# jirsat/wavenets

Measured on NVIDIA B200. Metric: audio samples/sec fwd+bwd WaveNet stack, higher is better.
Workload: dtype bf16

## Files before the change

### include/wavenet_b200.h

```cpp
#ifndef WAVENET_B200_H_
#define WAVENET_B200_H_

#include <stddef.h>
#include <stdint.h>

#ifdef __cplusplus
extern "C" {
#endif

typedef struct wn_handle wn_handle;

enum wn_status {
  WN_OK = 0,
  WN_ERR_VALUE = -1,
  WN_ERR_UNSUPPORTED = -2,
  WN_ERR_CUDA = -3,
  WN_ERR_STATE = -4
};

enum wn_activation { WN_ACT_LINEAR = 0, WN_ACT_RELU = 1, WN_ACT_LEAKY_RELU = 2, WN_ACT_TANH = 3, WN_ACT_SIGMOID = 4 };
enum wn_sampling { WN_CATEGORICAL = 0, WN_LOGISTIC = 1, WN_GAUSSIAN = 2 };
enum wn_precision {
  WN_FP32 = 0,
  WN_BF16 = 1
// ... 80 lines not shown
int wn_forward_ex(wn_handle* h, const float* x_dev, const float* cond_dev, int B, int T, int training, float* out_dev, void* stream);

int wn_loss_fn(wn_handle* h, const void* target_dev, int target_is_int64, const float* pred_dev, int B, int T, float* out_dev, void* stream);

int wn_train_step(wn_handle* h, const float* frames_dev, const float* cond_dev, int B, int T,
                  int n_replicas, float* loss_dev, void* stream);
int wn_test_step(wn_handle* h, const float* frames_dev, const float* cond_dev, int B, int T,
                 int n_replicas, float* loss_dev, void* stream);
int wn_train_step_host(wn_handle* h, const float* frames_host, const float* cond_host, int B, int T,
                       int n_replicas, float* loss_host);

int wn_nccl_unique_id(uint8_t* id128);
int wn_comm_init(wn_handle* h, const uint8_t* id128, int nranks, int rank);
int wn_comm_attach(wn_handle* h, void* nccl_comm , int nranks, int rank);
int wn_comm_fuse_allreduce(wn_handle* h, int on);
int wn_allreduce_grads(wn_handle* h, void* stream);
const char* wn_nccl_info(void);

int wn_layer_forward(wn_handle* h, int block, const float* x_dev, const float* cond_dev, int B, int T,
                     float* x_out_dev, float* skip_dev, void* stream);
int wn_layer_forward_ex(wn_handle* h, int block, const float* x_dev, const float* cond_dev, int B, int T, int training,
                        float* x_out_dev, float* skip_dev, void* stream);
int wn_layer_backward(wn_handle* h, int block, const float* dx_out_dev, const float* dskip_dev,
                      float* dx_dev, float* dcond_dev, void* stream);

int wn_debug_tensor(wn_handle* h, const char* name, int index, float* out_host, int64_t capacity);
int wn_debug_conv_gemm(const void* a_bf16_dev, int lda, int B, int T, int nseg, const int* shifts, int K,
                       const void* w_bf16_dev, int N, int N16, int tile, float* out_dev, void* stream);
int wn_debug_wgrad(const void* a_bf16_dev, int lda, const void* g_bf16_dev, int ldg, int B, int T, int nseg,
                   const int* shifts, int K, int N, float* out_dev, void* stream);
// ... 21 lines not shown
```

### wavenets_b200/_lib.py

```python
from __future__ import annotations

import ctypes as C
import os

WN_MAX_LIST = 8
WN_MAX_DILATIONS = 512

WN_OK, WN_ERR_VALUE, WN_ERR_UNSUPPORTED, WN_ERR_CUDA, WN_ERR_STATE = 0, -1, -2, -3, -4
ACTIVATIONS = {None: 0, 'linear': 0, 'relu': 1, 'leaky_relu': 2, 'tanh': 3, 'sigmoid': 4}
SAMPLING = {'categorical': 0, 'logistic': 1, 'gaussian': 2}
PRECISION = {'fp32': 0, 'float32': 0, 'bf16': 1, 'bfloat16': 1}

EXPORTS = [
  'wn_create', 'wn_destroy', 'wn_last_error', 'wn_receptive_field', 'wn_dilation', 'wn_num_params',
  'wn_param_count', 'wn_param_info', 'wn_params_dev', 'wn_grads_dev', 'wn_set_param', 'wn_get_param',
  'wn_get_grad', 'wn_params_changed', 'wn_quantize', 'wn_forward', 'wn_train_step', 'wn_test_step',
  'wn_train_step_host', 'wn_layer_forward', 'wn_layer_backward', 'wn_last_launch_count',
  'wn_fused_forward_blocks', 'wn_grouped_wgrad_tiles', 'wn_stack_forward_layers', 'wn_profile_begin', 'wn_profile_end', 'wn_profile_get', 'wn_build_info', 'wn_set_dropout_masks', 'wn_set_dropout_seed', 'wn_layer_forward_ex', 'wn_num_frames', 'wn_preprocess_frames', 'wn_inverse_mu_law', 'wn_one_hot', 'wn_sample_waveform', 'wn_sample_last_step', 'wn_generate', 'wn_adam_init', 'wn_clip_grads', 'wn_adam_step', 'wn_adam_state', 'wn_debug_conv_gemm', 'wn_debug_wgrad', 'wn_debug_bench',
  'wn_forward_ex', 'wn_loss_fn', 'wn_adam_restore', 'wn_nccl_unique_id', 'wn_comm_init', 'wn_comm_attach', 'wn_comm_fuse_allreduce',
  'wn_allreduce_grads', 'wn_nccl_info', 'wn_grouped_wgrad_info', 'wn_debug_tensor', 'wn_stack_backward_layers',
  'wn_allreduce_buckets',
]


class WnConfig(C.Structure):
  _fields_ = [
    ('kernel_size', C.c_int32), ('channels', C.c_int32), ('blocks', C.c_int32), ('layers_per_block', C.c_int32),
    ('activation', C.c_int32), ('conditioning', C.c_int32), ('n_mapping', C.c_int32),
    ('mapping_layers', C.c_int32 * WN_MAX_LIST), ('mapping_activation', C.c_int32), ('cond_in', C.c_int32),
    ('dilation_bound', C.c_int32), ('num_mixtures', C.c_int32), ('sampling_function', C.c_int32), ('bits', C.c_int32),
    ('skip_channels', C.c_int32), ('dilation_channels', C.c_int32), ('use_residual', C.c_int32), ('use_skip', C.c_int32),
    ('n_final', C.c_int32), ('final_layers_channels', C.c_int32 * WN_MAX_LIST),
    ('l2_reg_factor', C.c_float), ('dropout', C.c_float),
    ('n_dilations', C.c_int32), ('dilations', C.c_int32 * WN_MAX_DILATIONS),
# ... 36 lines not shown
  lib.wn_grads_dev.argtypes = [vp]
  lib.wn_grads_dev.restype = vp
  lib.wn_set_param.argtypes = [vp, i32, vp]
  lib.wn_get_param.argtypes = [vp, i32, vp]
  lib.wn_get_grad.argtypes = [vp, i32, vp]
  lib.wn_params_changed.argtypes = [vp, vp]
  lib.wn_quantize.argtypes = [vp, vp, i64, i32, vp]
  lib.wn_forward.argtypes = [vp, vp, vp, i32, i32, vp, vp]
  lib.wn_forward_ex.argtypes = [vp, vp, vp, i32, i32, i32, vp, vp]
  lib.wn_loss_fn.argtypes = [vp, vp, i32, vp, i32, i32, vp, vp]
  lib.wn_adam_restore.argtypes = [vp, vp, vp, i64]
  lib.wn_nccl_unique_id.argtypes = [vp]
  lib.wn_comm_init.argtypes = [vp, vp, i32, i32]
  lib.wn_comm_attach.argtypes = [vp, vp, i32, i32]
  lib.wn_comm_fuse_allreduce.argtypes = [vp, i32]
  lib.wn_allreduce_grads.argtypes = [vp, vp]
  lib.wn_nccl_info.restype = C.c_char_p
  lib.wn_train_step.argtypes = [vp, vp, vp, i32, i32, i32, vp, vp]
  lib.wn_test_step.argtypes = [vp, vp, vp, i32, i32, i32, vp, vp]
  lib.wn_train_step_host.argtypes = [vp, vp, vp, i32, i32, i32, vp]
  lib.wn_layer_forward.argtypes = [vp, i32, vp, vp, i32, i32, vp, vp, vp]
  lib.wn_layer_forward_ex.argtypes = [vp, i32, vp, vp, i32, i32, i32, vp, vp, vp]
  lib.wn_layer_backward.argtypes = [vp, i32, vp, vp, vp, vp, vp]
  lib.wn_last_launch_count.argtypes = [vp]
  lib.wn_last_launch_count.restype = i64
  lib.wn_fused_forward_blocks.argtypes = [vp]
  lib.wn_grouped_wgrad_tiles.argtypes = [vp, C.POINTER(C.c_int)]
  lib.wn_stack_forward_layers.argtypes = [vp]
  lib.wn_stack_backward_layers.argtypes = [vp]
  lib.wn_allreduce_buckets.argtypes = [vp]
# ... 46 lines not shown
```

### wavenets_b200/build.py

```python
from __future__ import annotations

import hashlib
import os
import subprocess
import sys

HERE = os.path.dirname(os.path.abspath(__file__))
CSRC = os.path.join(HERE, 'csrc')
LIB = os.path.join(HERE, 'libwavenet_b200.so')
STAMP = os.path.join(HERE, '.libwavenet_b200.stamp')
FLAVOURS = {'': [], 'precise': ['-DWN_PRECISE_MATH'], 'tl': ['-DTC_TIMELINE']}

SOURCES = ['wn_api.cu']
HEADERS = ['common.cuh', 'generate.cuh', 'epilogues.cuh', 'gemm_simt.cuh', 'gemm_tc.cuh', 'gemm_tc_block.cuh', 'gemm_tc_wgroup.cuh', 'gemm_tc_stack.cuh', 'gemm_tc_stack_bwd.cuh', 'tc_common.cuh', 'tc_epilogues.cuh', 'kernels_misc.cuh', 'nccl_dl.cuh',
           os.path.join('..', '..', 'include', 'wavenet_b200.h')]

NVCC_FLAGS = [
  '-gencode', 'arch=compute_100a,code=sm_100a', '-lineinfo', '-O3', '-std=c++17',
  '-Xcompiler', '-fPIC', '-shared', '--expt-relaxed-constexpr',
  '-Xptxas', '-v', '-ldl',
]


def _flags(flavour: str = ''):
  return NVCC_FLAGS + FLAVOURS[flavour] + os.environ.get('WN_NVCC_EXTRA', '').split()


def lib_path(flavour: str = '') -> str:
  return LIB if not flavour else os.path.join(HERE, f'libwavenet_b200_{flavour}.so')
# ... 39 lines not shown
```

### wavenets_b200/csrc/wn_api.cu

```cuda
#include <cuda_runtime.h>
#include <math.h>
#include <stdarg.h>
#include <stdio.h>
#include <stdlib.h>
#include <string.h>

#include <algorithm>
#include <string>
#include <vector>

#include "../../include/wavenet_b200.h"
#include "common.cuh"
#include "epilogues.cuh"
#include "gemm_simt.cuh"
#include "gemm_tc.cuh"
#include "gemm_tc_block.cuh"
#include "gemm_tc_wgroup.cuh"
#include "gemm_tc_stack.cuh"
#include "gemm_tc_stack_bwd.cuh"
#include "kernels_misc.cuh"
#include "generate.cuh"
#include "nccl_dl.cuh"

static thread_local char g_err[512] = "";
static void set_err(const char* fmt, ...) {
  va_list ap;
  va_start(ap, fmt);
  vsnprintf(g_err, sizeof(g_err), fmt, ap);
  va_end(ap);
}
extern "C" const char* wn_last_error(void) { return g_err; }
extern "C" const char* wn_build_info(void) {
  return "libwavenet_b200 sm_100a; fp32 FFMA tier + bf16 tcgen05/TMEM/TMA tier; built " __DATE__ " " __TIME__;
}
// ... 140 lines not shown
  size_t prof_used = 0;
  long long prof_launches = 0;
  TmapCache tmaps;
  struct StepGraph { const float* frames; const float* cond; int B, T, nrep; float* loss; bool train; int seen; long long launches; cudaGraphExec_t exec; };
  std::vector<StepGraph> graphs;
  int use_graphs = 1;
  cudaEvent_t ev_in = nullptr, ev_out = nullptr;
  cudaStream_t side_stream = nullptr;
  std::vector<cudaEvent_t> ev_blk_in, ev_blk_dz, ev_blk_done;
  int use_side = 1;
  int use_res_gemm = 1;
  int use_fused_fwd = 1;
  int stack_fwd_layers = 0;
  int use_stack_fwd = 1;
  std::vector<TcStackPlan> stack_plans;
  int use_stack_bwd = 2, stack_bwd_layers = 0;
  std::vector<TcStackBwdPlan> stack_bwd_plans;
  int tile_gate_bwd = 0, tile_dgrad = 0;
  int fused_fwd_launches = 0;
  int use_group_wgrad = 0;
  void* dz_all = nullptr;
  void* dx_all = nullptr;
  void* do_all = nullptr;
  std::vector<std::vector<void*>> dp_keep;
  struct WgPlan { int B, T; bool drop; bool sb; int nb; TcWgGroupPlan plan; };
  std::vector<WgPlan> wg_plans;
  std::vector<TcWgJobDesc> wg_jobs;
  int dskip_l2_last = 0;
  int wg_last_tiles = 0, wg_last_side = 0;
  int wg_last_partials = 0;
// ... 408 lines not shown
  cudaMemset(h->d_grads, 0, (size_t)h->n_scalars * 4);
  cudaMemset(h->pack.base, 0, pack_bytes);
  cudaMemset(h->ws.base, 0, ws_bytes);
  cudaMallocHost(&h->pin_frames, (size_t)h->maxB * (h->maxT + 1) * 4);
  cudaMallocHost(&h->pin_cond, (size_t)h->maxB * (c.cond_in > 0 ? c.cond_in : 1) * 4);
  cudaMallocHost(&h->pin_loss, 16);
  cudaStreamCreateWithFlags(&h->own_stream, cudaStreamNonBlocking);
  cudaEventCreateWithFlags(&h->ev_in, cudaEventDisableTiming);
  cudaEventCreateWithFlags(&h->ev_out, cudaEventDisableTiming);
  { const char* e = getenv("WN_CUDA_GRAPH"); if (e && e[0] == '0') h->use_graphs = 0; }
  { const char* e = getenv("WN_SIDE_STREAM"); if (e && e[0] == '0') h->use_side = 0; }
  if (env_res && env_res[0] == '0') h->use_res_gemm = 0;
  { const char* e = getenv("WN_TC_FUSED_FWD"); if (e && e[0] == '0') h->use_fused_fwd = 0; }
  { const char* e = getenv("WN_TC_STACK_FWD"); if (e && e[0] == '0') h->use_stack_fwd = 0; }
  { const char* e = getenv("WN_TC_STACK_BWD"); if (e) h->use_stack_bwd = atoi(e); }
  { const char* e = getenv("WN_TC_TILE_GATE_BWD"); if (e) h->tile_gate_bwd = atoi(e); }
  { const char* e = getenv("WN_TC_TILE_DGRAD"); if (e) h->tile_dgrad = atoi(e); }
  { const char* e = getenv("WN_TC_MERGED_FINISH"); if (e && e[0] == '1') h->use_merged_finish = 1; }
  { const char* e = getenv("WN_TC_BALANCE_GRID"); if (e) g_tc_balance_env = atoi(e); }
  { const char* e = getenv("WN_TC_DSKIP_LAST"); if (e) h->dskip_l2_last = atoi(e); }
  cudaStreamCreateWithFlags(&h->side_stream, cudaStreamNonBlocking);
  cudaEventCreateWithFlags(&h->ev_wg_side, cudaEventDisableTiming);
  {
    int lo = 0, hi = 0;
    cudaDeviceGetStreamPriorityRange(&lo, &hi);
    if (cudaStreamCreateWithPriority(&h->comm_stream, cudaStreamNonBlocking, hi) != cudaSuccess) {
      cudaGetLastError();
      cudaStreamCreateWithFlags(&h->comm_stream, cudaStreamNonBlocking);
    }
  }
// ... 640 lines not shown
    }
  }
  if (!stacked)
  for (int l = 0; l < h->L; ++l) {
    RET(block_forward<T>(h, st, l, cur, c.conditioning != 0, B, Tn));
    cur = h->xout[l];
  }
  const void* head_in = cur;
  int head_w = h->R;
  if (c.use_skip) {
    OuterLabel ol(h, "skip_sum");
    RET((skip_gemm<T, T>(h, st, 0, h->L, (T*)h->skipsum, h->Sp, h->bskip_sum, B, Tn)));
    head_in = h->skipsum;
    head_w = h->Sp;
  }
  OuterLabel ol_head(h, "head_fwd");
  for (size_t i = 0; i < h->head.size(); ++i) {
    const ConvP& hc = h->head[i];
    const bool last = i + 1 == h->head.size();
    GemmH g;
    g.B = B; g.T = Tn; g.N = hc.cout; g.nseg = 1;
    g.seg[0] = SegH{head_in, head_w, 0, hc.cin};
    fill_w(g, hc, false);
    if (!last) {
      typename EpiBiasActRes<T, T, sizeof(T) == 2>::Params ep{};
      ep.out = (T*)h->hact[i]; ep.ldo = hc.cout; ep.bias = P_(h, hc.b_idx); ep.act = c.activation; ep.N = hc.cout; ep.vec = vec_ok<T>(hc.cout);
      RET((run_conv_gemm<T, EpiBiasActRes<T, T, sizeof(T) == 2>>(h, st, CLS_GEMM, g, ep)));
      head_in = h->hact[i];
      head_w = hc.cout;
    } else {
      typename EpiBiasActRes<T, float, sizeof(T) == 2>::Params ep{};
      ep.out = h->logits; ep.ldo = h->ldl; ep.bias = P_(h, hc.b_idx); ep.act = ACT_LINEAR; ep.N = hc.cout; ep.vec = vec_ok<float>(h->ldl);
      RET((run_conv_gemm<T, EpiBiasActRes<T, float, sizeof(T) == 2>>(h, st, CLS_GEMM, g, ep)));
    }
  }
  return WN_OK;
}

template <class T>
static int loss_forward(wn_handle* h, cudaStream_t st, const float* frames, int B, int Tn, float scale, bool want_grad, float* probs, float* loss_out) {
  const wn_config& c = h->cfg;
  const long long rows = (long long)B * Tn;
  int nparts;
  {
    OuterLabel ol(h, "loss");
    LaunchScope ls(h, st, CLS_LOSS);
    if (c.sampling_function == WN_CATEGORICAL) {
      nparts = cdiv(rows, 8);
      if (h->Cout == 256 && h->ldl == 256 && h->ldd % 4 == 0)
        softmax_ce_reg_kernel<T, 2><<<nparts, 256, 0, st>>>(h->logits, frames, Tn, rows, c.bits, scale, want_grad ? (T*)h->dlogits : nullptr, h->ldd, probs,
                                                           loss_out ? h->loss_partial : nullptr);
      else
        softmax_ce_kernel<T><<<nparts, 256, 0, st>>>(h->logits, h->Cout, frames, Tn, rows, c.bits, scale, want_grad ? (T*)h->dlogits : nullptr, h->ldd,
                                                    probs, loss_out ? h->loss_partial : nullptr);
    } else {
      mixture_loss_launch<T>(st, &nparts, h->logits, h->ldl, c.num_mixtures, frames, Tn, rows, c.bits, c.sampling_function == WN_GAUSSIAN ? 2 : 1, scale,
                             want_grad ? (T*)h->dlogits : nullptr, h->ldd, loss_out ? h->loss_partial : nullptr, Tn + 1, 1, nullptr);
    }
  }
// ... 396 lines not shown
    g.seg[0] = SegH{dcur, dw, 0, (sizeof(T) == 2 && i + 1 == (int)h->head.size()) ? h->ldd : hc.cout};
    fill_w(g, hc, true);
    typename EpiActBwd<T, T>::Params ep{};
    ep.N = hc.cin; ep.add = nullptr;
    void* dst;
    if (i > 0) {
      dst = (dcur == h->dhA) ? h->dhB : h->dhA;
      ep.out = (T*)dst; ep.ldo = hc.cin; ep.y = (const T*)h->hact[i - 1]; ep.ldy = hc.cin; ep.act = c.activation; ep.vec = vec_ok<T>(hc.cin);
    } else if (cat) {
      dst = (T*)h->dcatA + h->R;
      ep.out = (T*)dst; ep.ldo = ldc; ep.y = nullptr; ep.act = ACT_LINEAR; ep.vec = vec_ok<T>(ldc);
    } else {
      dst = c.use_skip ? h->dskip : (group ? dx_of(h->L - 1) : h->dxA);
      ep.out = (T*)dst; ep.ldo = hc.cin; ep.y = nullptr; ep.act = ACT_LINEAR; ep.vec = vec_ok<T>(hc.cin);
    }
    RET((run_conv_gemm<T, EpiActBwd<T, T>>(h, st, CLS_GEMM, g, ep)));
    dcur = dst;
    dw = hc.cin;
  }
  const void* dxout;
  int ld_dx;
  if (cat) {
    CK(cudaMemcpy2DAsync((T*)h->dcatB + h->R, (size_t)ldc * sizeof(T), (const T*)h->dcatA + h->R, (size_t)ldc * sizeof(T), (size_t)h->S * sizeof(T),
                         (size_t)B * Tn, cudaMemcpyDeviceToDevice, st));
    const void* cur = nullptr;
    void* nxt = h->dcatB;
    for (int l = h->L - 1; l >= 0; --l) {
      const void* x_in = l > 0 ? h->xout[l - 1] : h->h0;
      const void* dsk = cur ? (const void*)((const T*)cur + h->R) : (const void*)((const T*)h->dcatA + h->R);
      BwdSide sd; const BwdSide* sdp = side_setup(h, st, l, use_side, &sd);
      RET(block_backward<T>(h, st, l, x_in, cur, ldc, dsk, ldc, nxt, ldc, B, Tn, l2coef, (l & 1) ? h->dz2 : h->dz, sdp));
// ... 464 lines not shown
                                       mse_dev ? h->loss_partial : nullptr);
  if (mse_dev) loss_finalize<<<1, 1024, 0, st>>>(h->loss_partial, nparts, 1.0f / (float)rows, nullptr, 0.f, mse_dev);
  CK(cudaGetLastError());
  return WN_OK;
}
extern "C" int wn_sample_waveform(wn_handle* h, const float* pred_dev, int B, int T, int deterministic, uint64_t seed, float* out_dev, void* stream) {
  RET(check_bt(h, B, T));
  if (!pred_dev || !out_dev || !h->cfg.has_head) { set_err("bad sample arguments"); return WN_ERR_VALUE; }
  CK(cudaSetDevice(h->cfg.device));
  return sample_common(h, pred_dev, h->Cout, 0, nullptr, B, T, deterministic, seed, out_dev, nullptr, (cudaStream_t)stream);
}
extern "C" int wn_sample_last_step(wn_handle* h, const float* frames_dev, int deterministic, uint64_t seed, float* out_dev, float* mse_dev, void* stream) {
  if (!h || !h->cfg.has_head || h->lastB < 1) { set_err("no train/test step to sample from"); return WN_ERR_STATE; }
  if (!out_dev) { set_err("bad sample arguments"); return WN_ERR_VALUE; }
  CK(cudaSetDevice(h->cfg.device));
  return sample_common(h, h->logits, h->ldl, 1, mse_dev ? frames_dev : nullptr, h->lastB, h->lastT, deterministic, seed, out_dev, mse_dev, (cudaStream_t)stream);
}

extern "C" int wn_adam_init(wn_handle* h, float lr, float beta1, float beta2, float eps, float clipnorm) {
  if (!h) { set_err("null handle"); return WN_ERR_VALUE; }
  if (lr < 0.f || beta1 < 0.f || beta1 >= 1.f || beta2 < 0.f || beta2 >= 1.f || eps <= 0.f || clipnorm < 0.f) { set_err("bad Adam hyper-parameters"); return WN_ERR_VALUE; }
  CK(cudaSetDevice(h->cfg.device));
  h->opt_lr = lr; h->opt_b1 = beta1; h->opt_b2 = beta2; h->opt_eps = eps; h->opt_clipnorm = clipnorm; h->opt_t = 0;
  const size_t bytes = (size_t)h->n_scalars * 4;
  if (!h->opt_m) {
    CK(cudaMalloc(&h->opt_m, bytes)); CK(cudaMalloc(&h->opt_v, bytes));
    std::vector<OptChunk> ch; std::vector<int> first;
    for (size_t v = 0; v < h->params.size(); ++v) {
      first.push_back((int)ch.size());
      for (long long o = 0; o < h->params[v].count; o += OPT_CHUNK)
// ... 208 lines not shown
}
extern "C" int wn_comm_attach(wn_handle* h, void* nccl_comm, int nranks, int rank) {
  if (!h || nranks < 1) { set_err("bad communicator arguments"); return WN_ERR_VALUE; }
  char err[256];
  if (nccl_comm && nccl_load(err, sizeof(err)) != 0) { set_err("%s", err); return WN_ERR_CUDA; }
  if (h->comm && h->comm_owned) g_nccl.CommDestroy(h->comm);
  h->comm = (wn_ncclComm_t)nccl_comm; h->comm_owned = false; h->comm_nranks = nccl_comm ? nranks : 1; h->comm_rank = rank;
  drop_graphs_fwd(h);
  return WN_OK;
}
extern "C" int wn_comm_fuse_allreduce(wn_handle* h, int on) {
  if (!h) { set_err("null handle"); return WN_ERR_VALUE; }
  if ((on != 0) != (h->ar_in_step != 0)) { h->ar_in_step = on ? 1 : 0; drop_graphs_fwd(h); }
  return WN_OK;
}
extern "C" int wn_allreduce_grads(wn_handle* h, void* stream) {
  if (!h) { set_err("null handle"); return WN_ERR_VALUE; }
  if (h->comm_nranks <= 1) return WN_OK;
  CK(cudaSetDevice(h->cfg.device));
  return allreduce_grads(h, (cudaStream_t)stream);
}
extern "C" const char* wn_nccl_info(void) {
  static char buf[400];
  char err[256];
  if (nccl_load(err, sizeof(err)) != 0) { snprintf(buf, sizeof(buf), "unavailable: %s", err); return buf; }
  int v = 0;
  if (g_nccl.GetVersion) g_nccl.GetVersion(&v);
  snprintf(buf, sizeof(buf), "NCCL %d from %s", v, g_nccl.where);
  return buf;
}

template <class T>
static int step_entry(wn_handle* h, const float* frames, const float* cond, int B, int Tn, int nrep, float* loss, cudaStream_t st, bool train) {
  const float scale = 1.0f / ((float)B * (float)nrep);
  h->drop_active = train && h->cfg.dropout > 0.f;
  draw_dropout_masks(h, st, B, Tn);
  RET(model_forward<T>(h, st, frames, Tn + 1, cond, B, Tn));
  RET(loss_forward<T>(h, st, frames, B, Tn, scale, train, nullptr, loss));
  if (train) {
    const float l2coef = h->cfg.l2_reg_factor > 0.f ? 2.0f * h->cfg.l2_reg_factor / (float)nrep : 0.f;
    h->ar_now = h->ar_in_step && h->comm && h->comm_nranks > 1 && nrep > 1;
    RET(model_backward<T>(h, st, frames, Tn + 1, cond, B, Tn, l2coef));
    if (h->ar_now) RET(allreduce_grads(h, st));
    h->ar_now = false;
  }
  return WN_OK;
}

static int step_common(wn_handle* h, const float* frames_dev, const float* cond_dev, int B, int T, int n_replicas, float* loss_dev, void* stream, bool train) {
  RET(check_bt(h, B, T));
  if (!h->cfg.has_head || !h->cfg.has_input_conv) { set_err("train/test step needs a full model handle"); return WN_ERR_STATE; }
  if (h->cfg.conditioning && !cond_dev) { set_err("Conditioning must be provided."); return WN_ERR_VALUE; }
  if (n_replicas < 1 || !frames_dev || !loss_dev) { set_err("bad step arguments"); return WN_ERR_VALUE; }
  if (train && h->cfg.dropout >= 1.f) { set_err("dropout must be < 1 for training"); return WN_ERR_VALUE; }
  CK(cudaSetDevice(h->cfg.device));
  cudaStream_t st = (cudaStream_t)stream;
  auto run = [&](cudaStream_t s) -> int {
    h->launches = 0;
    return h->cfg.precision == WN_BF16 ? step_entry<bf16>(h, frames_dev, cond_dev, B, T, n_replicas, loss_dev, s, train)
                                       : step_entry<float>(h, frames_dev, cond_dev, B, T, n_replicas, loss_dev, s, train);
  };
  if (h->use_graphs && h->prof_tag == 0) {
    wn_handle::StepGraph* sg = nullptr;
    for (auto& g : h->graphs)
      if (g.frames == frames_dev && g.cond == cond_dev && g.B == B && g.T == T && g.nrep == n_replicas && g.loss == loss_dev && g.train == train) { sg = &g; break; }
    if (!sg) {
      if (h->graphs.size() >= 8) { for (auto& g : h->graphs) if (g.exec) cudaGraphExecDestroy(g.exec); h->graphs.clear(); }
      h->graphs.push_back({frames_dev, cond_dev, B, T, n_replicas, loss_dev, train, 0, 0, nullptr});
      sg = &h->graphs.back();
    }
    const bool legacy = st == nullptr || st == cudaStreamLegacy;
    cudaStream_t gs = legacy ? h->own_stream : st;
    if (sg->seen >= 1 && !sg->exec) {
      cudaGraph_t graph = nullptr;
      if (cudaStreamBeginCapture(gs, cudaStreamCaptureModeThreadLocal) == cudaSuccess) {
        int r = run(gs);
// ... 5 lines not shown
          h->use_graphs = 0;
          cudaGetLastError();
        }
        if (graph) cudaGraphDestroy(graph);
      } else {
        h->use_graphs = 0;
        cudaGetLastError();
      }
    }
    if (sg->exec) {
      if (legacy) { CK(cudaEventRecord(h->ev_in, st)); CK(cudaStreamWaitEvent(gs, h->ev_in, 0)); }
      CK(cudaGraphLaunch(sg->exec, gs));
      if (legacy) { CK(cudaEventRecord(h->ev_out, gs)); CK(cudaStreamWaitEvent(st, h->ev_out, 0)); }
      h->launches = sg->launches;
      h->lastB = B; h->lastT = T;
      return WN_OK;
    }
    sg->seen++;
  }
  RET(run(st));
  CK(cudaGetLastError());
  h->lastB = B; h->lastT = T;
  return WN_OK;
}

extern "C" int wn_train_step(wn_handle* h, const float* frames_dev, const float* cond_dev, int B, int T, int n_replicas, float* loss_dev, void* stream) {
  return step_common(h, frames_dev, cond_dev, B, T, n_replicas, loss_dev, stream, true);
}
extern "C" int wn_test_step(wn_handle* h, const float* frames_dev, const float* cond_dev, int B, int T, int n_replicas, float* loss_dev, void* stream) {
  return step_common(h, frames_dev, cond_dev, B, T, n_replicas, loss_dev, stream, false);
}

extern "C" int wn_train_step_host(wn_handle* h, const float* frames_host, const float* cond_host, int B, int T, int n_replicas, float* loss_host) {
  RET(check_bt(h, B, T));
  if (!frames_host || !loss_host) { set_err("bad step arguments"); return WN_ERR_VALUE; }
  CK(cudaSetDevice(h->cfg.device));
  cudaStream_t st = h->own_stream;
// ... 126 lines not shown
  const size_t rows_cap = (size_t)h->maxB * h->maxT;
  const bool bf = h->cfg.precision == WN_BF16;
  const size_t es = bf ? 2 : 4;
  const std::string n(name);
  const void* src = nullptr; int width = 0, ld = 0; bool f32 = false;
  const bool lok = index >= 0 && index < h->L;
  if (n == "h0") { src = h->h0; width = ld = h->R; }
  else if (n == "z" && lok) { src = h->zbuf[index]; width = ld = 2 * h->D; }
  else if (n == "g" && lok) { src = (const char*)h->G_all + (size_t)index * rows_cap * h->D * es; width = ld = h->D; }
  else if (n == "xout" && lok) { src = h->xout[index]; width = ld = h->R; }
  else if (n == "skipsum") { src = h->skipsum; width = ld = h->Sp; }
  else if (n == "hact" && index >= 0 && index < (int)h->hact.size()) { src = h->hact[index]; width = ld = h->head[index].cout; }
  else if (n == "act" && index >= 0 && index / 16 < h->L && index % 16 < (int)h->acts[index / 16].size()) {
    src = h->acts[index / 16][index % 16]; width = ld = h->D;
  }
  else if (n == "logits") { src = h->logits; width = h->Cout; ld = h->ldl; f32 = true; }
  else if (n == "dlogits") { src = h->dlogits; width = h->Cout; ld = h->ldd; }
  else if (n == "dskip") { src = h->dskip; width = ld = h->Sp; }
  else if (n == "dz" && lok && h->dz_all) { src = (const char*)h->dz_all + (size_t)index * rows_cap * 2 * h->D * es; width = ld = 2 * h->D; }
  else if (n == "dx" && lok && h->dx_all) { src = (const char*)h->dx_all + (size_t)index * rows_cap * h->R * es; width = ld = h->R; }
  if (!src || rows < 1) { set_err("debug_tensor: no tensor '%s'[%d] in this handle / step", name, index); return WN_ERR_STATE; }
  if ((long long)capacity < rows * width) { set_err("debug_tensor: capacity %lld < %lld", (long long)capacity, rows * width); return WN_ERR_VALUE; }
  const size_t e2 = f32 ? 4 : es;
  std::vector<char> tmp((size_t)rows * ld * e2);
  CK(cudaMemcpy(tmp.data(), src, tmp.size(), cudaMemcpyDeviceToHost));
  for (long long r = 0; r < rows; ++r)
    for (int c = 0; c < width; ++c) {
      const char* p = tmp.data() + ((size_t)r * ld + c) * e2;
      float v;
      if (e2 == 4) memcpy(&v, p, 4);
      else { uint16_t u; memcpy(&u, p, 2); uint32_t w = (uint32_t)u << 16; memcpy(&v, &w, 4); }
// ... 139 lines not shown
```

### wavenets_b200/model.py

```python
from __future__ import annotations

import ctypes as C
import math
import warnings
from typing import Optional

import numpy as np
import torch

from . import _lib
from ._engine import Handle, as_dev
from .layers import WaveNetLayer
from .metrics import Mean


class _PendingLogs:

  def __init__(self, model, slot, event):
    self._model, self._slot, self._event, self._out = model, slot, event, None

  def result(self):
    if self._out is None:
      self._event.synchronize()
      m = self._model
# ... 75 lines not shown
    self.dilations = [kernel_size ** (i % max_power) for i in range(layers_per_block * blocks)]
    self.receptive_field = 1 + sum(self.dilations) * (kernel_size - 1) + 1

    self._act = _lib.activation_code(activation)
    self._map_act = _lib.activation_code(mapping_activation)
    self.optimizer = None
    self.built = False
    self._handle: Optional[Handle] = None
    self._pending_weights = None
    self._staging = {}
    self._metrics_from_compilation = []
    self.loss_tracker = None
    self.reg_loss = None
    self.last_step_logs = {}
    self._sample_seed, self._sample_calls = 0x42, 0
    self._pin_logs, self._pin_events, self._pending_slot = None, None, 0
    self._last_frames, self._last_rows = None, 0
    self.n_replicas = 1
    self.replica_rank = 0
    self._process_group = None
    self._comm = None
    self._dropout_seed = 0x243F6A8885A308D3
    self._ar_fused = False

  def compile(self, **kwargs):
    if 'loss' in kwargs:
      raise ValueError('Loss must be set in the model init function.')
    self.optimizer = kwargs.get('optimizer', None)
    self._metrics_from_compilation = list(kwargs.get('metrics') or [])
    self.loss_tracker = Mean(name='loss')
# ... 199 lines not shown
    dev = torch.device('cuda', self.device_index)
    if len(x.shape) == 3 and x.shape[2] != 1:
      raise ValueError('input must be (batch, samples, 1)')
    B, T = int(x.shape[0]), int(x.shape[1]) - 1
    frames = self._stage('frames', x, (B, T + 1), dev)
    cond = self._stage('cond', cond, (B, int(cond.shape[-1])), dev) if cond is not None else None
    self._ensure_built(frames[:, :-1], cond)
    h = self.handle
    self._last_frames, self._last_rows = frames, B * T
    fn = h.lib.wn_train_step if train else h.lib.wn_test_step
    if train and self._comm is not None:
      fuse = not (self.optimizer is not None and getattr(self.optimizer, 'clipnorm', None))
      if fuse != self._ar_fused:
        _lib.check(h.lib.wn_comm_fuse_allreduce(h.h, 1 if fuse else 0))
        self._ar_fused = fuse
    _lib.check(fn(h.h, h.ptr(frames), h.ptr(cond), B, T, self.n_replicas, h.ptr(h._loss), h.stream_ptr()))
    clip = train and self.optimizer is not None and getattr(self.optimizer, 'clipnorm', None)
    if clip:
      self.optimizer.clip(self)
    if train and self.n_replicas > 1:
      if self._comm is not None:
        if not self._ar_fused:
          _lib.check(h.lib.wn_allreduce_grads(h.h, h.stream_ptr()))
      elif self._process_group is not None:
        torch.distributed.all_reduce(h.flat_grads, op=torch.distributed.ReduceOp.SUM, group=self._process_group)
    return h._loss[:2]

  def train_step(self, data):
    loss = self._step(data, True)
    if self.optimizer is not None:
# ... 163 lines not shown
```

Before: 11.03 million.

## Fuse head forward, categorical loss and head backward into one tcgen05 kernel

Adds a persistent 2-CTA cluster kernel that runs the three 1x1 head convolutions, the softmax cross-entropy loss with its gradient, and the backward head GEMMs in one launch. Intermediates stay in TMEM and shared memory, and only bf16 outputs are stored through TMA. This removes separate GEMM and loss launches and the fp32 logits round trip. Logits are no longer written by default; they are recomputed lazily when sampling, debugging or metrics need them, which adds state-tracking complexity.

```diff
diff --git a/include/wavenet_b200.h b/include/wavenet_b200.h
--- a/include/wavenet_b200.h
+++ b/include/wavenet_b200.h
@@ -118,6 +118,7 @@
 int wn_comm_init(wn_handle* h, const uint8_t* id128, int nranks, int rank);
 int wn_comm_attach(wn_handle* h, void* nccl_comm , int nranks, int rank);
 int wn_comm_fuse_allreduce(wn_handle* h, int on);
+int wn_keep_logits(wn_handle* h, int on);
 int wn_allreduce_grads(wn_handle* h, void* stream);
 const char* wn_nccl_info(void);
 
diff --git a/wavenets_b200/_lib.py b/wavenets_b200/_lib.py
--- a/wavenets_b200/_lib.py
+++ b/wavenets_b200/_lib.py
@@ -17,7 +17,7 @@
   'wn_get_grad', 'wn_params_changed', 'wn_quantize', 'wn_forward', 'wn_train_step', 'wn_test_step',
   'wn_train_step_host', 'wn_layer_forward', 'wn_layer_backward', 'wn_last_launch_count',
   'wn_fused_forward_blocks', 'wn_grouped_wgrad_tiles', 'wn_stack_forward_layers', 'wn_profile_begin', 'wn_profile_end', 'wn_profile_get', 'wn_build_info', 'wn_set_dropout_masks', 'wn_set_dropout_seed', 'wn_layer_forward_ex', 'wn_num_frames', 'wn_preprocess_frames', 'wn_inverse_mu_law', 'wn_one_hot', 'wn_sample_waveform', 'wn_sample_last_step', 'wn_generate', 'wn_adam_init', 'wn_clip_grads', 'wn_adam_step', 'wn_adam_state', 'wn_debug_conv_gemm', 'wn_debug_wgrad', 'wn_debug_bench',
-  'wn_forward_ex', 'wn_loss_fn', 'wn_adam_restore', 'wn_nccl_unique_id', 'wn_comm_init', 'wn_comm_attach', 'wn_comm_fuse_allreduce',
+  'wn_forward_ex', 'wn_loss_fn', 'wn_adam_restore', 'wn_nccl_unique_id', 'wn_comm_init', 'wn_comm_attach', 'wn_comm_fuse_allreduce', 'wn_keep_logits',
   'wn_allreduce_grads', 'wn_nccl_info', 'wn_grouped_wgrad_info', 'wn_debug_tensor', 'wn_stack_backward_layers',
   'wn_allreduce_buckets',
 ]
@@ -84,6 +84,7 @@
   lib.wn_comm_init.argtypes = [vp, vp, i32, i32]
   lib.wn_comm_attach.argtypes = [vp, vp, i32, i32]
   lib.wn_comm_fuse_allreduce.argtypes = [vp, i32]
+  lib.wn_keep_logits.argtypes = [vp, i32]
   lib.wn_allreduce_grads.argtypes = [vp, vp]
   lib.wn_nccl_info.restype = C.c_char_p
   lib.wn_train_step.argtypes = [vp, vp, vp, i32, i32, i32, vp, vp]
diff --git a/wavenets_b200/build.py b/wavenets_b200/build.py
--- a/wavenets_b200/build.py
+++ b/wavenets_b200/build.py
@@ -12,7 +12,7 @@
 FLAVOURS = {'': [], 'precise': ['-DWN_PRECISE_MATH'], 'tl': ['-DTC_TIMELINE']}
 
 SOURCES = ['wn_api.cu']
-HEADERS = ['common.cuh', 'generate.cuh', 'epilogues.cuh', 'gemm_simt.cuh', 'gemm_tc.cuh', 'gemm_tc_block.cuh', 'gemm_tc_wgroup.cuh', 'gemm_tc_stack.cuh', 'gemm_tc_stack_bwd.cuh', 'tc_common.cuh', 'tc_epilogues.cuh', 'kernels_misc.cuh', 'nccl_dl.cuh',
+HEADERS = ['common.cuh', 'generate.cuh', 'epilogues.cuh', 'gemm_simt.cuh', 'gemm_tc.cuh', 'gemm_tc_block.cuh', 'gemm_tc_wgroup.cuh', 'gemm_tc_stack.cuh', 'gemm_tc_stack_bwd.cuh', 'gemm_tc_head.cuh', 'tc_common.cuh', 'tc_epilogues.cuh', 'kernels_misc.cuh', 'nccl_dl.cuh',
            os.path.join('..', '..', 'include', 'wavenet_b200.h')]
 
 NVCC_FLAGS = [
diff --git a/wavenets_b200/csrc/gemm_tc_head.cuh b/wavenets_b200/csrc/gemm_tc_head.cuh
--- /dev/null
+++ b/wavenets_b200/csrc/gemm_tc_head.cuh
@@ -0,0 +1,365 @@
+#pragma once
+#include "gemm_tc_block.cuh"
+#include "kernels_misc.cuh"
+
+struct TcHeadMaps {
+  CUtensorMap m[13];
+};
+
+struct TcHeadParams {
+  int B, T, tiles_t, num_mtiles;
+  const float* bias[3];
+  int act;
+  const float* frames; int bits; float scale;
+  float* loss_partial;
+  const bf16* hA; const bf16* hB;
+  unsigned long long pol_s, pol_w, pol_o;
+};
+
+struct TcHeadCfg {
+  static constexpr int BM = 128;
+  static constexpr int W_BYTES = 128 * 64 * 2;
+  static constexpr int STAGES = 4;
+  static constexpr int BUF_BYTES = BM * 256 * 2;
+  static constexpr int SMEM_BYTES = STAGES * W_BYTES + 2 * BUF_BYTES + 3 * 256 * 4 + 256;
+  static_assert(SMEM_BYTES <= 232448, "head kernel does not fit shared memory");
+};
+
+__device__ __forceinline__ void tc_head_put16(uint8_t* buf, int row, int ch, const float* v) {
+  uint8_t* gs = buf + (ch >> 6) * (TcHeadCfg::BUF_BYTES / 4) + row * 128;
+  const uint32_t j0 = (uint32_t)((ch & 63) >> 3), sw = (uint32_t)(row & 7);
+  uint4 a, c;
+  a.x = pack_bf16x2(v[0], v[1]); a.y = pack_bf16x2(v[2], v[3]); a.z = pack_bf16x2(v[4], v[5]); a.w = pack_bf16x2(v[6], v[7]);
+  c.x = pack_bf16x2(v[8], v[9]); c.y = pack_bf16x2(v[10], v[11]); c.z = pack_bf16x2(v[12], v[13]); c.w = pack_bf16x2(v[14], v[15]);
+  *reinterpret_cast<uint4*>(gs + ((j0 ^ sw) << 4)) = a;
+  *reinterpret_cast<uint4*>(gs + (((j0 + 1) ^ sw) << 4)) = c;
+}
+
+__device__ __forceinline__ float tc_head_butterfly(float* p) {
+#pragma unroll
+  for (int o = 16; o > 0; o >>= 1)
+#pragma unroll
+    for (int L = 0; L < o; ++L) p[L] = p[L] + p[L + o];
+  return p[0];
+}
+
+__global__ void __launch_bounds__(384, 1) tc_head_kernel(const __grid_constant__ TcHeadMaps maps, const TcHeadParams p) {
+  using Cfg = TcHeadCfg;
+  constexpr int STAGES = Cfg::STAGES;
+  extern __shared__ __align__(1024) uint8_t smem_head[];
+  uint8_t* smem = smem_head;
+  if ((smem_u32(smem) & 1023u) != 0u) { if (threadIdx.x == 0) printf("libwavenet_b200: dynamic shared memory is not 1024-byte aligned\n"); __trap(); }
+  uint8_t* bufs = smem + STAGES * Cfg::W_BYTES;
+  float* bias_s = (float*)(bufs + 2 * Cfg::BUF_BYTES);
+  uint64_t* full_bar = (uint64_t*)(bias_s + 3 * 256);
+  uint64_t* empty_bar = full_bar + STAGES;
+  uint64_t* sfull = empty_bar + STAGES;
+  uint64_t* tfull = sfull + 2;
+  uint64_t* ready = tfull + 2;
+  uint64_t* bfree = ready + 2;
+  uint32_t* tmem_ptr = (uint32_t*)(bfree + 2);
+
+  const int warp = threadIdx.x >> 5, lane = threadIdx.x & 31;
+  const uint32_t crank = cluster_ctarank();
+  const bool leader = crank == 0;
+  const int pair = (int)blockIdx.x >> 1, npairs = (int)gridDim.x >> 1;
+  const int n_mt = pair < p.num_mtiles ? (p.num_mtiles - pair + npairs - 1) / npairs : 0;
+  const int n_rounds = (n_mt + 1) / 2;
+
+  if (warp == 0 && lane == 0)
+    for (int i = 0; i < 7; ++i) tma_prefetch_desc(&maps.m[i]);
+  if (warp == 1 && lane == 0) {
+    for (int i = 0; i < STAGES; ++i) { mbar_init(&full_bar[i], 1); mbar_init(&empty_bar[i], 1); }
+    for (int i = 0; i < 2; ++i) { mbar_init(&sfull[i], 1); mbar_init(&tfull[i], 1); mbar_init(&ready[i], 2); mbar_init(&bfree[i], 1); }
+    mbar_fence_init();
+  }
+  if (warp == 2) tmem_alloc_pair<512>(tmem_ptr);
+  tc_fence_before();
+  __syncthreads();
+  cluster_sync_all();
+  tc_fence_after();
+  const uint32_t tmem_base = *tmem_ptr;
+  pdl_launch_dependents();
+  pdl_wait();
+  for (int i = threadIdx.x; i < 3 * 256; i += blockDim.x) bias_s[i] = __ldg(p.bias[i >> 8] + (i & 255));
+  __syncthreads();
+
+  auto tile_of = [&](int j, int& b, int& t0) {
+    const int mt = pair + j * npairs;
+    b = mt / p.tiles_t; t0 = (mt % p.tiles_t) * 256 + (int)crank * Cfg::BM;
+  };
+
+  if (warp == 0) {
+    if (lane == 0) {
+      int stage = 0; uint32_t phase = 0;
+      for (int r = 0; r < n_rounds; ++r) {
+        for (int pr = 0; pr < 6; ++pr) {
+          for (int s = 0; s < 2; ++s) {
+            const int j = 2 * r + s;
+            if (j >= n_mt) continue;
+            if (pr == 0) {
+              if (r > 0) mbar_wait(&bfree[s], (uint32_t)((r - 1) & 1));
+              int b, t0; tile_of(j, b, t0);
+              uint8_t* buf = bufs + s * Cfg::BUF_BYTES;
+              if (leader) mbar_expect_tx(&sfull[s], 2 * Cfg::BUF_BYTES);
+#pragma unroll
+              for (int kb = 0; kb < 4; ++kb) tma_load_3d_pair_h(buf + kb * (Cfg::BUF_BYTES / 4), &maps.m[0], &sfull[s], kb * 64, t0, b, p.pol_s);
+            }
+            for (int kb = 0; kb < 4; ++kb) {
+              mbar_wait(&empty_bar[stage], phase ^ 1);
+              if (leader) mbar_expect_tx(&full_bar[stage], 2 * Cfg::W_BYTES);
+              tma_load_2d_pair_h(smem + stage * Cfg::W_BYTES, &maps.m[1 + pr], &full_bar[stage], kb * 64, (int)crank * 128, p.pol_w);
+              if (++stage == STAGES) { stage = 0; phase ^= 1; }
+            }
+          }
+        }
+      }
+    }
+  } else if (warp == 1) {
+    if (leader) {
+      constexpr uint32_t idesc = umma_idesc_bf16(256, 256, 0, 0);
+      int stage = 0; uint32_t phase = 0;
+      for (int r = 0; r < n_rounds; ++r) {
+        for (int pr = 0; pr < 6; ++pr) {
+          for (int s = 0; s < 2; ++s) {
+            const int j = 2 * r + s;
+            if (j >= n_mt) continue;
+            if (pr == 0) {
+              mbar_wait(&sfull[s], (uint32_t)(r & 1));
+              if (r > 0) mbar_wait(&ready[s], 1u);
+            } else {
+              mbar_wait(&ready[s], (uint32_t)((pr - 1) & 1));
+            }
+            tc_fence_after();
+            const uint32_t d_tmem = tmem_base + (uint32_t)(s * 256);
+            const uint32_t a0 = smem_u32(bufs + s * Cfg::BUF_BYTES);
+            for (int kb = 0; kb < 4; ++kb) {
+              mbar_wait(&full_bar[stage], phase);
+              tc_fence_after();
+              if (elect_one()) {
+                const uint64_t adesc = umma_smem_desc(a0 + (uint32_t)kb * (uint32_t)(Cfg::BUF_BYTES / 4), 16, 1024);
+                const uint64_t bdesc = umma_smem_desc(smem_u32(smem + stage * Cfg::W_BYTES), 16, 1024);
+#pragma unroll
+                for (int k = 0; k < 4; ++k) umma_bf16_pair(d_tmem, adesc + (uint64_t)(2 * k), bdesc + (uint64_t)(2 * k), idesc, (kb | k) != 0);
+                umma_commit_pair(&empty_bar[stage]);
+                if (kb == 3) umma_commit_pair(&tfull[s]);
+              }
+              __syncwarp();
+              if (++stage == STAGES) { stage = 0; phase ^= 1; }
+            }
+          }
+        }
+      }
+    }
+  } else if (warp >= 4) {
+    const int s = (warp - 4) >> 2;
+    const int quarter = warp & 3;
+    const int row = quarter * 32 + lane;
+    const bool issuer = (warp & 3) == 0 && lane == 0;
+    const int bar_id = 1 + s;
+    uint8_t* buf = bufs + s * Cfg::BUF_BYTES;
+    const uint32_t tacc = tmem_base + (uint32_t)(s * 256) + ((uint32_t)(quarter * 32) << 16);
+    for (int j = s; j < n_mt; j += 2) {
+      int b, t0; tile_of(j, b, t0);
+      const int t = t0 + row;
+      const bool valid = t < p.T;
+      const long long grow = (long long)b * p.T + t;
+      for (int e = 0; e < 6; ++e) {
+        mbar_wait(&tfull[s], (uint32_t)(e & 1));
+        tc_fence_after();
+        if (issuer) {
+          if (e == 3) { bulk_wait_group<0>(); asm volatile("fence.proxy.async.global;" ::: "memory"); }
+          else bulk_wait_group_read<0>();
+        }
+        named_bar_sync(bar_id, 128);
+        if (e < 2) {
+          const float* bs = bias_s + e * 256;
+#pragma unroll 1
+          for (int c = 0; c < 256; c += 16) {
+            float v[16], bb[16];
+            tmem_ld16(tacc + (uint32_t)c, v);
+            ld_bias16(bs + c, bb);
+#pragma unroll
+            for (int i = 0; i < 16; ++i) v[i] += bb[i];
+            if (p.act != ACT_LINEAR) wn_act16<true>(p.act, v);
+            tc_head_put16(buf, row, c, v);
+          }
+        } else if (e == 2) {
+          const float* bs = bias_s + 512;
+          int idx = -1;
+          if (valid) idx = wn_quantize_idx(p.frames[(long long)b * (p.T + 1) + t + 1], p.bits);
+          float m = -INFINITY, ly = 0.f;
+#pragma unroll
+          for (int ci = 0; ci < 16; ++ci) {
+            float v[16], bb[16];
+            tmem_ld16(tacc + (uint32_t)(ci * 16), v);
+            ld_bias16(bs + ci * 16, bb);
+#pragma unroll
+            for (int i = 0; i < 16; ++i) {
+              v[i] += bb[i];
+              m = fmaxf(m, v[i]);
+              if (ci * 16 + i == idx) ly = v[i];
+            }
+          }
+          float part[32];
+          float emin = INFINITY;
+#pragma unroll
+          for (int ci = 0; ci < 16; ++ci) {
+            float v[16], bb[16];
+            tmem_ld16(tacc + (uint32_t)(ci * 16), v);
+            ld_bias16(bs + ci * 16, bb);
+#pragma unroll
+            for (int i = 0; i < 16; ++i) { v[i] = expf((v[i] + bb[i]) - m); emin = fminf(emin, v[i]); }
+#pragma unroll
+            for (int q = 0; q < 4; ++q) {
+              const float qs = v[4 * q] + v[4 * q + 1] + v[4 * q + 2] + v[4 * q + 3];
+              const int L = (ci & 7) * 4 + q;
+              if (ci < 8) part[L] = 0.f + qs; else part[L] = part[L] + qs;
+            }
+          }
+          const float ssum = tc_head_butterfly(part);
+          const float inv = 1.0f / ssum;
+          const bool clipped = emin * inv < WN_CE_EPS || inv > 1.0f - WN_CE_EPS;
+          WnCeClip cc;
+          cc.S_inv = 1.f; cc.dot = 0.f; cc.y_coef = 1.f;
+          float delta = 0.f, pm = 0.f;
+          if (__any_sync(0xffffffffu, clipped)) {
+            float dp[32], pp[32];
+#pragma unroll
+            for (int L = 0; L < 32; ++L) { dp[L] = 0.f; pp[L] = 0.f; }
+#pragma unroll
+            for (int ci = 0; ci < 16; ++ci) {
+              float v[16], bb[16];
+              tmem_ld16(tacc + (uint32_t)(ci * 16), v);
+              ld_bias16(bs + ci * 16, bb);
+#pragma unroll
+              for (int i = 0; i < 16; ++i) {
+                const float pv = expf((v[i] + bb[i]) - m) * inv;
+                const bool in = pv >= WN_CE_EPS && pv <= 1.0f - WN_CE_EPS;
+                const int L = (ci & 7) * 4 + (i >> 2);
+                dp[L] += fminf(fmaxf(pv, WN_CE_EPS), 1.0f - WN_CE_EPS) - pv;
+                pp[L] += in ? pv : 0.f;
+              }
+            }
+            delta = tc_head_butterfly(dp);
+            pm = tc_head_butterfly(pp);
+          }
+          float loss = 0.f;
+          if (valid) {
+            loss = (m + logf(ssum)) - ly;
+            if (clipped) loss = wn_ce_clip(cc, delta, pm, expf(ly - m) * inv, loss);
+          } else if (clipped) {
+            wn_ce_clip(cc, delta, pm, 0.5f, 0.f);
+          }
+#pragma unroll 1
+          for (int ci = 0; ci < 16; ++ci) {
+            float v[16], bb[16];
+            tmem_ld16(tacc + (uint32_t)(ci * 16), v);
+            ld_bias16(bs + ci * 16, bb);
+            float d[16];
+#pragma unroll
+            for (int i = 0; i < 16; ++i) {
+              const float pv = expf((v[i] + bb[i]) - m) * inv;
+              const int c = ci * 16 + i;
+              d[i] = clipped ? wn_ce_clip_grad(cc, pv, c == idx) * p.scale : (pv - (c == idx ? 1.0f : 0.0f)) * p.scale;
+            }
+            tc_head_put16(buf, row, ci * 16, d);
+          }
+          float tot = 0.f;
+#pragma unroll
+          for (int k = 0; k < 8; ++k) tot += __shfl_sync(0xffffffffu, loss, (lane & ~7) + k);
+          if ((lane & 7) == 0 && valid) p.loss_partial[grow >> 3] = tot;
+        } else {
+          const bf16* y = e == 3 ? p.hB : (e == 4 ? p.hA : nullptr);
+          const bool agrad = y != nullptr && p.act != ACT_LINEAR;
+          const bf16* yrow = agrad ? y + (valid ? grow : 0) * 256 : nullptr;
+#pragma unroll 1
+          for (int c = 0; c < 256; c += 16) {
+            float v[16];
+            tmem_ld16(tacc + (uint32_t)c, v);
+            if (agrad) {
+              float yv[16];
+              const uint4 q0 = __ldcg(reinterpret_cast<const uint4*>(yrow + c)), q1 = __ldcg(reinterpret_cast<const uint4*>(yrow + c + 8));
+              const uint32_t w[8] = {q0.x, q0.y, q0.z, q0.w, q1.x, q1.y, q1.z, q1.w};
+#pragma unroll
+              for (int k = 0; k < 8; ++k) { yv[2 * k] = __uint_as_float(w[k] << 16); yv[2 * k + 1] = __uint_as_float(w[k] & 0xffff0000u); }
+              wn_act_grad16(p.act, yv, v);
+            }
+            tc_head_put16(buf, row, c, v);
+          }
+        }
+        tc_fence_before();
+        fence_proxy_async();
+        named_bar_sync(bar_id, 128);
+        if (issuer) {
+          const CUtensorMap* om = &maps.m[7 + e];
+#pragma unroll
+          for (int kb = 0; kb < 4; ++kb) tma_store_3d_h(buf + kb * (Cfg::BUF_BYTES / 4), om, kb * 64, t0, b, p.pol_o);
+          bulk_commit_group();
+          if (e == 5) { bulk_wait_group_read<0>(); mbar_arrive(&bfree[s]); }
+          if (leader) mbar_arrive(&ready[s]);
+          else mbar_arrive_remote(&ready[s], 0u);
+        }
+        __syncwarp();
+      }
+    }
+    if (issuer) bulk_wait_group<0>();
+  }
+  tc_fence_before();
+  __syncthreads();
+  cluster_sync_all();
+  if (warp == 2) tmem_dealloc_pair<512>(tmem_base);
+}
+
+struct TcHeadDesc {
+  int B, T, act, bits;
+  const bf16* skipsum;
+  const bf16* Wf[3]; int kf[3];
+  const bf16* Wb[3]; int kb[3];
+  const float* bias[3];
+  bf16* hA; bf16* hB; bf16* dlogits; bf16* dhB; bf16* dhA; bf16* dskip;
+  const float* frames; float scale; float* loss_partial;
+};
+
+static inline int tc_head_launch(TmapCache& tc, cudaStream_t st, const TcHeadDesc& d) {
+  using Cfg = TcHeadCfg;
+  TcHeadMaps maps;
+  const CUtensorMap* ms = tc_slab_map(tc, d.skipsum, 256, 256, d.T, d.B);
+  if (!ms) return -10;
+  maps.m[0] = *ms;
+  for (int i = 0; i < 6; ++i) {
+    const bf16* W = i < 3 ? d.Wf[i] : d.Wb[5 - i];
+    const int k = i < 3 ? d.kf[i] : d.kb[5 - i];
+    uint64_t wd[2] = {(uint64_t)k, 256}, ws[1] = {(uint64_t)k * 2};
+    uint32_t wb[2] = {64, 128};
+    const CUtensorMap* mw = tc.get(W, 2, wd, ws, wb);
+    if (!mw) return -10;
+    maps.m[1 + i] = *mw;
+  }
+  bf16* outs[6] = {d.hA, d.hB, d.dlogits, d.dhB, d.dhA, d.dskip};
+  for (int i = 0; i < 6; ++i) {
+    const CUtensorMap* mo = tc_slab_map(tc, outs[i], 256, 256, d.T, d.B);
+    if (!mo) return -10;
+    maps.m[7 + i] = *mo;
+  }
+  TcHeadParams p{};
+  p.B = d.B; p.T = d.T; p.tiles_t = (d.T + 255) / 256; p.num_mtiles = d.B * p.tiles_t;
+  for (int i = 0; i < 3; ++i) p.bias[i] = d.bias[i];
+  p.act = d.act; p.frames = d.frames; p.bits = d.bits; p.scale = d.scale; p.loss_partial = d.loss_partial;
+  p.hA = d.hA; p.hB = d.hB;
+  p.pol_s = tc_policy(TC_L2_FIRST); p.pol_w = tc_policy(TC_L2_LAST); p.pol_o = tc_policy(TC_L2_NORMAL);
+  static unsigned long long attr_devs = 0ull;
+  if (tc_first_use_on_device(&attr_devs)) {
+    cudaError_t e = cudaFuncSetAttribute(tc_head_kernel, cudaFuncAttributeMaxDynamicSharedMemorySize, Cfg::SMEM_BYTES);
+    if (e != cudaSuccess) { snprintf(g_tc_err, sizeof(g_tc_err), "cudaFuncSetAttribute(smem=%d): %s", Cfg::SMEM_BYTES, cudaGetErrorString(e)); return -12; }
+  }
+  const int pairs = tc_num_sms() / 2;
+  const int grid = (p.num_mtiles < pairs ? p.num_mtiles : pairs) * 2;
+  cudaLaunchConfig_t cfg{};
+  cfg.gridDim = dim3(grid); cfg.blockDim = dim3(384); cfg.dynamicSmemBytes = Cfg::SMEM_BYTES; cfg.stream = st;
+  cudaLaunchAttribute attr[2];
+  cfg.attrs = attr; cfg.numAttrs = tc_launch_attrs(attr, 2);
+  cudaError_t e = cudaLaunchKernelEx(&cfg, tc_head_kernel, maps, p);
+  if (e != cudaSuccess) { snprintf(g_tc_err, sizeof(g_tc_err), "head launch: %s", cudaGetErrorString(e)); return -13; }
+  return 0;
+}
diff --git a/wavenets_b200/csrc/wn_api.cu b/wavenets_b200/csrc/wn_api.cu
--- a/wavenets_b200/csrc/wn_api.cu
+++ b/wavenets_b200/csrc/wn_api.cu
@@ -18,6 +18,7 @@
 #include "gemm_tc_wgroup.cuh"
 #include "gemm_tc_stack.cuh"
 #include "gemm_tc_stack_bwd.cuh"
+#include "gemm_tc_head.cuh"
 #include "kernels_misc.cuh"
 #include "generate.cuh"
 #include "nccl_dl.cuh"
@@ -188,6 +189,10 @@
   int stack_fwd_layers = 0;
   int use_stack_fwd = 1;
   std::vector<TcStackPlan> stack_plans;
+  int use_head_fused = 1;
+  bool head_fused_now = false;
+  bool logits_stale = false;
+  bool keep_logits = false;
   int use_stack_bwd = 2, stack_bwd_layers = 0;
   std::vector<TcStackBwdPlan> stack_bwd_plans;
   int tile_gate_bwd = 0, tile_dgrad = 0;
@@ -626,6 +631,7 @@
   { const char* e = getenv("WN_TC_FUSED_FWD"); if (e && e[0] == '0') h->use_fused_fwd = 0; }
   { const char* e = getenv("WN_TC_STACK_FWD"); if (e && e[0] == '0') h->use_stack_fwd = 0; }
   { const char* e = getenv("WN_TC_STACK_BWD"); if (e) h->use_stack_bwd = atoi(e); }
+  { const char* e = getenv("WN_TC_HEAD_FUSED"); if (e && e[0] == '0') h->use_head_fused = 0; }
   { const char* e = getenv("WN_TC_TILE_GATE_BWD"); if (e) h->tile_gate_bwd = atoi(e); }
   { const char* e = getenv("WN_TC_TILE_DGRAD"); if (e) h->tile_dgrad = atoi(e); }
   { const char* e = getenv("WN_TC_MERGED_FINISH"); if (e && e[0] == '1') h->use_merged_finish = 1; }
@@ -1296,6 +1302,7 @@
     head_in = h->skipsum;
     head_w = h->Sp;
   }
+  if (h->head_fused_now) return WN_OK;
   OuterLabel ol_head(h, "head_fwd");
   for (size_t i = 0; i < h->head.size(); ++i) {
     const ConvP& hc = h->head[i];
@@ -1319,12 +1326,42 @@
   return WN_OK;
 }
 
+static int head_logits(wn_handle* h, cudaStream_t st, int B, int Tn) {
+  const ConvP& hc = h->head.back();
+  GemmH g;
+  g.B = B; g.T = Tn; g.N = hc.cout; g.nseg = 1;
+  g.seg[0] = SegH{h->hact.back(), hc.cin, 0, hc.cin};
+  fill_w(g, hc, false);
+  EpiBiasActRes<bf16, float, true>::Params ep{};
+  ep.out = h->logits; ep.ldo = h->ldl; ep.bias = P_(h, hc.b_idx); ep.act = ACT_LINEAR; ep.N = hc.cout; ep.vec = vec_ok<float>(h->ldl);
+  return run_conv_gemm<bf16, EpiBiasActRes<bf16, float, true>>(h, st, CLS_GEMM, g, ep);
+}
+
 template <class T>
 static int loss_forward(wn_handle* h, cudaStream_t st, const float* frames, int B, int Tn, float scale, bool want_grad, float* probs, float* loss_out) {
   const wn_config& c = h->cfg;
   const long long rows = (long long)B * Tn;
   int nparts;
-  {
+  if (h->head_fused_now) {
+    if constexpr (sizeof(T) == 2) {
+      OuterLabel ol(h, "head");
+      LaunchScope ls(h, st, CLS_GEMM);
+      nparts = cdiv(rows, 8);
+      TcHeadDesc d{};
+      d.B = B; d.T = Tn; d.act = c.activation; d.bits = c.bits;
+      d.skipsum = (const bf16*)h->skipsum;
+      for (int i = 0; i < 3; ++i) {
+        const ConvP& hc = h->head[i];
+        d.Wf[i] = hc.Wf16; d.kf[i] = hc.Kf16; d.Wb[i] = hc.Wb16; d.kb[i] = rup(hc.Kb16, 64); d.bias[i] = P_(h, hc.b_idx);
+      }
+      d.hA = (bf16*)h->hact[0]; d.hB = (bf16*)h->hact[1]; d.dlogits = (bf16*)h->dlogits;
+      d.dhB = (bf16*)h->dhA; d.dhA = (bf16*)h->dhB; d.dskip = (bf16*)h->dskip;
+      d.frames = frames; d.scale = scale; d.loss_partial = h->loss_partial;
+      const int r = tc_head_launch(h->tmaps, st, d);
+      if (r != 0) { set_err("head launch failed (%d): %s", r, tc_last_error()); return WN_ERR_CUDA; }
+      if (h->keep_logits) RET(head_logits(h, st, B, Tn));
+    }
+  } else {
     OuterLabel ol(h, "loss");
     LaunchScope ls(h, st, CLS_LOSS);
     if (c.sampling_function == WN_CATEGORICAL) {
@@ -1751,7 +1788,7 @@
       dst = c.use_skip ? h->dskip : (group ? dx_of(h->L - 1) : h->dxA);
       ep.out = (T*)dst; ep.ldo = hc.cin; ep.y = nullptr; ep.act = ACT_LINEAR; ep.vec = vec_ok<T>(hc.cin);
     }
-    RET((run_conv_gemm<T, EpiActBwd<T, T>>(h, st, CLS_GEMM, g, ep)));
+    if (!h->head_fused_now) RET((run_conv_gemm<T, EpiActBwd<T, T>>(h, st, CLS_GEMM, g, ep)));
     dcur = dst;
     dw = hc.cin;
   }
@@ -2246,6 +2283,7 @@
   if (!h || !h->cfg.has_head || h->lastB < 1) { set_err("no train/test step to sample from"); return WN_ERR_STATE; }
   if (!out_dev) { set_err("bad sample arguments"); return WN_ERR_VALUE; }
   CK(cudaSetDevice(h->cfg.device));
+  if (h->logits_stale) RET(head_logits(h, (cudaStream_t)stream, h->lastB, h->lastT));
   return sample_common(h, h->logits, h->ldl, 1, mse_dev ? frames_dev : nullptr, h->lastB, h->lastT, deterministic, seed, out_dev, mse_dev, (cudaStream_t)stream);
 }
 
@@ -2484,6 +2522,11 @@
   if ((on != 0) != (h->ar_in_step != 0)) { h->ar_in_step = on ? 1 : 0; drop_graphs_fwd(h); }
   return WN_OK;
 }
+extern "C" int wn_keep_logits(wn_handle* h, int on) {
+  if (!h) { set_err("null handle"); return WN_ERR_VALUE; }
+  if ((on != 0) != h->keep_logits) { h->keep_logits = on != 0; drop_graphs_fwd(h); }
+  return WN_OK;
+}
 extern "C" int wn_allreduce_grads(wn_handle* h, void* stream) {
   if (!h) { set_err("null handle"); return WN_ERR_VALUE; }
   if (h->comm_nranks <= 1) return WN_OK;
@@ -2500,11 +2543,23 @@
   return buf;
 }
 
+static bool head_fused_ok(wn_handle* h, int B, int Tn) {
+  const wn_config& c = h->cfg;
+  if (!h->use_head_fused || tc_cta_group() != 2) return false;
+  if (c.sampling_function != WN_CATEGORICAL || h->Cout != 256 || h->ldl != 256 || h->ldd != 256) return false;
+  if (!c.use_skip || h->Sp != 256 || h->dcatA != nullptr || h->head.size() != 3 || Tn % 8 != 0) return false;
+  for (const ConvP& hc : h->head)
+    if (hc.K != 1 || hc.cin != 256 || hc.cout != 256 || !hc.Wf16 || !hc.Wb16 || hc.Kf16 != 256 || hc.N16 < 256 || hc.C16 < 256) return false;
+  return (long long)B * Tn > 0;
+}
+
 template <class T>
 static int step_entry(wn_handle* h, const float* frames, const float* cond, int B, int Tn, int nrep, float* loss, cudaStream_t st, bool train) {
   const float scale = 1.0f / ((float)B * (float)nrep);
   h->drop_active = train && h->cfg.dropout > 0.f;
   draw_dropout_masks(h, st, B, Tn);
+  h->head_fused_now = sizeof(T) == 2 && train && head_fused_ok(h, B, Tn);
+  struct Reset { wn_handle* h; ~Reset() { h->head_fused_now = false; } } reset{h};
   RET(model_forward<T>(h, st, frames, Tn + 1, cond, B, Tn));
   RET(loss_forward<T>(h, st, frames, B, Tn, scale, train, nullptr, loss));
   if (train) {
@@ -2530,6 +2585,7 @@
     return h->cfg.precision == WN_BF16 ? step_entry<bf16>(h, frames_dev, cond_dev, B, T, n_replicas, loss_dev, s, train)
                                        : step_entry<float>(h, frames_dev, cond_dev, B, T, n_replicas, loss_dev, s, train);
   };
+  const bool fused_head = train && h->cfg.precision == WN_BF16 && head_fused_ok(h, B, T) && !h->keep_logits;
   if (h->use_graphs && h->prof_tag == 0) {
     wn_handle::StepGraph* sg = nullptr;
     for (auto& g : h->graphs)
@@ -2565,6 +2621,7 @@
       if (legacy) { CK(cudaEventRecord(h->ev_out, gs)); CK(cudaStreamWaitEvent(st, h->ev_out, 0)); }
       h->launches = sg->launches;
       h->lastB = B; h->lastT = T;
+      h->logits_stale = fused_head;
       return WN_OK;
     }
     sg->seen++;
@@ -2572,6 +2629,7 @@
   RET(run(st));
   CK(cudaGetLastError());
   h->lastB = B; h->lastT = T;
+  h->logits_stale = fused_head;
   return WN_OK;
 }
 
@@ -2728,7 +2786,7 @@
   else if (n == "act" && index >= 0 && index / 16 < h->L && index % 16 < (int)h->acts[index / 16].size()) {
     src = h->acts[index / 16][index % 16]; width = ld = h->D;
   }
-  else if (n == "logits") { src = h->logits; width = h->Cout; ld = h->ldl; f32 = true; }
+  else if (n == "logits") { if (h->logits_stale) { RET(head_logits(h, 0, h->lastB, h->lastT)); CK(cudaDeviceSynchronize()); } src = h->logits; width = h->Cout; ld = h->ldl; f32 = true; }
   else if (n == "dlogits") { src = h->dlogits; width = h->Cout; ld = h->ldd; }
   else if (n == "dskip") { src = h->dskip; width = ld = h->Sp; }
   else if (n == "dz" && lok && h->dz_all) { src = (const char*)h->dz_all + (size_t)index * rows_cap * 2 * h->D * es; width = ld = 2 * h->D; }
diff --git a/wavenets_b200/model.py b/wavenets_b200/model.py
--- a/wavenets_b200/model.py
+++ b/wavenets_b200/model.py
@@ -113,6 +113,7 @@
     self.reg_loss = None
     self.last_step_logs = {}
     self._sample_seed, self._sample_calls = 0x42, 0
+    self._keep_logits = False
     self._pin_logs, self._pin_events, self._pending_slot = None, None, 0
     self._last_frames, self._last_rows = None, 0
     self.n_replicas = 1
@@ -342,6 +343,10 @@
       if fuse != self._ar_fused:
         _lib.check(h.lib.wn_comm_fuse_allreduce(h.h, 1 if fuse else 0))
         self._ar_fused = fuse
+    keep = bool(self._metrics_from_compilation)
+    if keep != self._keep_logits:
+      _lib.check(h.lib.wn_keep_logits(h.h, 1 if keep else 0))
+      self._keep_logits = keep
     _lib.check(fn(h.h, h.ptr(frames), h.ptr(cond), B, T, self.n_replicas, h.ptr(h._loss), h.stream_ptr()))
     clip = train and self.optimizer is not None and getattr(self.optimizer, 'clipnorm', None)
     if clip:
```

After: 11.10 million, median of 6. No clear change (+0.7%).
